# utiasASRL/mm_masking

Hardware: AMD Instinct MI355X
Metric: scan-pairs/s (mask-CNN + 10-iter dICP fwd+bwd) (higher is better)
Workload: dtype bf16; 1 GPU; BASELINE configs[2]: train_icp_weights step fwd+bwd, batch=32 per GPU, 10 dICP iters, point-to-plane Huber, dim=2; 400x3360 polar radar -> GO-CFAR + peaks + polar->Cartesian 640x640 -> U-Net (hand-written NHWC bf16 MFMA kernels, fp32 masters) -> dICP (fp32 points, fp64 normal equations) -> rot+trans+mask_pts loss -> Adam; batch_per_gpu=32, global_batch=32, scan_pts_pad=5120, map_pts=20000, map_pts_pad=20480, icp_iters=10, parallelism=dp1, scene_density=survey (SURVEY.md 8d: 3 500-5 000 valid scan points of 5 120)

## Files before the change

### mm_masking_amd/csrc/mmk_unet.hip

```cpp
#include <math.h>
#include <stdlib.h>

#include <algorithm>
#include <type_traits>

#include "mmk_common.h"
#include "mmk_unet_shared.h"

namespace {

using namespace mmku;

__device__ __forceinline__ unsigned cvt_pk_bf16(float lo, float hi)
{
    unsigned r;
    asm("v_cvt_pk_bf16_f32 %0, %1, %2" : "=v"(r) : "v"(lo), "v"(hi));
    return r;
}
__device__ __forceinline__ unsigned pk_relu_bf16(unsigned x)
{
    unsigned r;
    asm("v_pk_max_i16 %0, %1, 0" : "=v"(r) : "v"(x));
    return r;
}
// ... 670 lines not shown

    float bs8[8];
    if constexpr (C8) {
#pragma unroll
        for (int r = 0; r < 8; ++r) {
            bs8[r] = a.bias ? a.bias[r] : 0.f;
            asm volatile("" : "+v"(bs8[r]));
        }
    }
    const float dk = dp.inv_keep;
    const unsigned thr1pk = ((unsigned)(dp.thr_s - 1 < -32768 ? -32768 : dp.thr_s - 1) & 0xffffu) * 0x00010001u;
#pragma unroll
    for (int m = 0; m < MT; ++m)
#pragma unroll
        for (int r = 0; r < 4; ++r) bs[m][r] *= dk;
    if constexpr (C8) {
#pragma unroll
        for (int r = 0; r < 8; ++r) bs8[r] *= dk;
    }

    MMK_RING_LOAD(0);
    MMK_RING_LOAD(1);
    MMK_RING_SINKS();
    if constexpr (RD > 2) {
        MMK_RING_LOAD(2);
        MMK_RING_SINKS();
    }
    cur_pix0 = s_pix0[0]; cur_ty0 = s_ty0[0]; cur_tx0 = s_tx0[0];
    if constexpr (POOL) cur_pp0 = s_pp0[0];
    MMK_RING_STORE(0, 0);
    MMK_RING_LOAD(0);
    MMK_RING_SINKS();

    int k0 = 0;
    {
#define STAGE_CHECKED 1
#define STAGE_SLOT 0
#include "mmk_conv_ring_stage.inc"
#undef STAGE_SLOT
#define STAGE_SLOT 1
#include "mmk_conv_ring_stage.inc"
#undef STAGE_SLOT
        if constexpr (RD > 2) {
#define STAGE_SLOT 2
#include "mmk_conv_ring_stage.inc"
#undef STAGE_SLOT
        }
#undef STAGE_CHECKED
    }
    for (k0 = RD; k0 + RD <= nt_blk; k0 += RD) {
#define STAGE_CHECKED 0
#define STAGE_SLOT 0
#include "mmk_conv_ring_stage.inc"
#undef STAGE_SLOT
#define STAGE_SLOT 1
#include "mmk_conv_ring_stage.inc"
#undef STAGE_SLOT
        if constexpr (RD > 2) {
#define STAGE_SLOT 2
#include "mmk_conv_ring_stage.inc"
#undef STAGE_SLOT
        }
#undef STAGE_CHECKED
    }
    {
#define STAGE_CHECKED 1
#define STAGE_SLOT 0
#include "mmk_conv_ring_stage.inc"
#undef STAGE_SLOT
        if constexpr (RD > 2) {
#define STAGE_SLOT 1
#include "mmk_conv_ring_stage.inc"
#undef STAGE_SLOT
        }
#undef STAGE_CHECKED
    }
ring_done:;
#ifdef MMK_DEEP_STAMPS
    if (tid == 0) { stamp_lds[16 + 6] = __builtin_amdgcn_s_memtime(); stamp_lds[16 + 7] = __builtin_amdgcn_s_memrealtime(); }
    __syncthreads();
    if (g_deep_stamp_buf != nullptr && blockIdx.y == 0 && blockIdx.x < 4096 && tid == 0) {
        unsigned long long *life = g_deep_stamp_buf + (size_t)64 * (4 * MMK_STAMP_STAGES * 8) + (size_t)blockIdx.x * 2;
        life[0] = stamp_lds[8 + 7];
        life[1] = stamp_lds[16 + 7];
    }
    if (g_deep_stamp_buf != nullptr && blockIdx.y == 0 && blockIdx.x < 64)
        for (int i = tid; i < 4 * MMK_STAMP_STAGES * 8; i += CONV_THREADS)
            g_deep_stamp_buf[(size_t)blockIdx.x * (4 * MMK_STAMP_STAGES * 8) + i] = stamp_lds[i];
#endif
#undef MMK_RING_LOAD
#undef MMK_RING_STORE
}

template <int CK, int CM, int RD, bool EPI, int POOL = 0, bool C8 = false, bool POOLG = false>
int launch_conv_ring(const ConvArgs &a, hipStream_t st)
{
#ifdef MMK_DEEP_STAMPS
    const size_t smem = (((size_t)2 * HT * WT * lds_pitch(CK) + (size_t)ksteps(CK) * (CM / 16) * 512) * sizeof(bf16) + 15) / 16 * 16 +
                        (size_t)4 * MMK_STAMP_STAGES * 8 * sizeof(unsigned long long);
#else
    const size_t smem = ((size_t)2 * HT * WT * lds_pitch(CK) + (size_t)ksteps(CK) * (CM / 16) * 512) * sizeof(bf16);
#endif
    constexpr auto kernel = conv3x3_ring_kernel<CK, CM, RD, EPI, POOL, C8, POOLG>;
    int per_cu = 0;
    MMK_CHECK_HIP(blocks_per_cu<kernel>(CONV_THREADS, smem, 8, &per_cu));
    const int groups = (a.COUT + CM - 1) / CM;
    const XcdGrid g = xcd_grid(a.B, a.H, a.W, TH, TW, groups, per_cu);
    hipLaunchKernelGGL(kernel, dim3(8 * g.nb, groups), dim3(CONV_THREADS), smem, st, a, g.total, g.per_xcd);
    MMK_LAUNCH_CHECK();
    return MMK_OK;
}

inline bool use_c8_epilogue()
{
    static int v = -1;
    if (v < 0) {
        const char *e = getenv("MMK_CONV_C8");
        v = (e && e[0] == '0') ? 0 : 1;
    }
    return v == 1;
}

template <int CK, int CM>
int launch_conv_ring_epi(const ConvArgs &a, hipStream_t st)
{
    constexpr int RD = CK <= 16 ? 3 : 2;
    constexpr int RDE = 2;
    const bool epi = a.o1.relu_src || a.o1.accumulate || (a.o2.C > 0 && (a.o2.relu_src || a.o2.accumulate));
    if (a.x1_pool_arg != nullptr) {
        if constexpr (CK == 32 && CM == 32) {
            if (epi && a.pool_y == nullptr) return launch_conv_ring<CK, CM, RDE, true, 0, false, true>(a, st);
        }
        mmk::set_error("mmk_conv3x3: x1_pool_arg is not supported for this layer (CIN=%d COUT=%d)", a.CIN, a.COUT);
        return MMK_ERR_ARG;
    }
    if (a.pool_y != nullptr) {
        if constexpr (CK == CM && (CK == 16 || CK == 32)) {
            if (!epi && a.o2.C == 0)
                return a.pool_arg != nullptr ? launch_conv_ring<CK, CM, RD, false, 2>(a, st) : launch_conv_ring<CK, CM, RD, false, 1>(a, st);
        }
        mmk::set_error("mmk_conv3x3: pool_y is not supported for this layer (see mmk_conv3x3_pool_fusable)");
        return MMK_ERR_ARG;
    }
    if constexpr (CM == 16) {
        if (a.COUT == 8 && a.o2.C == 0 && use_c8_epilogue())
            return epi ? launch_conv_ring<CK, CM, RDE, true, false, true>(a, st) : launch_conv_ring<CK, CM, RD, false, false, true>(a, st);
    }
    return epi ? launch_conv_ring<CK, CM, RDE, true>(a, st) : launch_conv_ring<CK, CM, RD, false>(a, st);
}


constexpr int DEEP_THREADS = 512;

template <int BM, int NT>
struct DeepCfg {
    static constexpr int WM = BM >= 128 ? 2 : 1;
    static constexpr int WN = 8 / WM;
    static constexpr int MT = BM / 16 / WM;
    static constexpr int MTB = BM / 16;
    static constexpr int TH = WN, TWD = NT * 16;
    static constexpr int HT = TH + 2, WT = TWD + 2;
    static constexpr int CK = 32, PK = 48, NS = 9, GPP = 4;
    static constexpr int NIN = HT * WT * GPP;
    static constexpr int NW = NS * MTB * 64;
    static constexpr int RIN = (NIN + DEEP_THREADS - 1) / DEEP_THREADS;
    static constexpr int RW = (NW + DEEP_THREADS - 1) / DEEP_THREADS;
    static constexpr size_t IN_BYTES = (size_t)HT * WT * PK * sizeof(bf16), W_BYTES = (size_t)NW * 8 * sizeof(bf16);
    static constexpr size_t smem_core(int wchunks) { return IN_BYTES + (size_t)wchunks * W_BYTES + BM * sizeof(float); }
#ifdef MMK_DEEP_STAMPS
    static constexpr size_t smem(int wchunks) { return (smem_core(wchunks) + 15) / 16 * 16 + (size_t)8 * MMK_STAMP_STAGES * 8 * sizeof(unsigned long long); }
#else
    static constexpr size_t smem(int wchunks) { return smem_core(wchunks); }
#endif
};

template <int BM, int NT>
XcdGrid deep_grid(int B, int H, int W, int cout)
{
    return xcd_grid(B, H, W, DeepCfg<BM, NT>::TH, DeepCfg<BM, NT>::TWD, (cout + BM - 1) / BM, 1);
}

template <int BM, int NT, bool LK = false, bool SUBW = false, int ROLE = 0, bool WRES = false, bool POOLG = false>
__global__ __launch_bounds__(DEEP_THREADS) void conv3x3_deep_kernel(const ConvArgs a, int total_tiles, int tiles_per_xcd)
{
    using C = DeepCfg<BM, NT>;
    constexpr int MT = C::MT, MTB = C::MTB, PK = C::PK, WT = C::WT, HT = C::HT, GPP = C::GPP;
    constexpr int NIN = C::NIN, NW = C::NW, RIN = C::RIN, RW = C::RW, NS = C::NS;
    constexpr bool R_FWD = ROLE == 1, R_BWD = ROLE == 2;
    static_assert(!(WRES && SUBW), "resident weights: the kernel's own packing only");
    extern __shared__ __attribute__((aligned(16))) unsigned char smem[];
    bf16 *in_tile = reinterpret_cast<bf16 *>(smem);
    bf16 *w_lds = in_tile + HT * WT * PK;

    const int tid = threadIdx.x, lane = tid & 63, wv = tid >> 6;
    const int wm = wv / C::WN, wn = wv % C::WN;
    const int tiles_x = (a.W + C::TWD - 1) / C::TWD, tiles_y = (a.H + C::TH - 1) / C::TH;
    const int tpi = tiles_x * tiles_y;
    const int group = blockIdx.y;
    const int nchunk = a.CIN / 32;
    const int wchunks = WRES ? nchunk : 1;

    const int xcd = blockIdx.x & 7, nb = gridDim.x >> 3;
    const int t_begin = xcd * tiles_per_xcd;
    const int t_end = (t_begin + tiles_per_xcd < total_tiles) ? t_begin + tiles_per_xcd : total_tiles;
    int tile = t_begin + (blockIdx.x >> 3);
    if (tile >= t_end) return;

    constexpr int RWL = WRES ? 0 : RW;
    constexpr int PHT = C::TH / 2 + 2, PWT = C::TWD / 2 + 2, NPIN = PHT * PWT * GPP;
    constexpr int NRIN = POOLG ? (NPIN + DEEP_THREADS - 1) / DEEP_THREADS : RIN;
    u32x4 rin[NRIN], rw[RW];
    unsigned rcd[POOLG ? NRIN : 1];
    const int Hp = a.H >> 1, Wp = a.W >> 1;
    int g_dy[RIN], g_dx[RIN], g_c[RIN], g_pix[RIN];
#pragma unroll
    for (int i = 0; i < RIN; ++i) {
        int g = tid + i * DEEP_THREADS;
        g = g < NIN ? g : NIN - 1;
        const int pix = g / GPP;
        g_dy[i] = pix / WT - 1;
        g_dx[i] = pix % WT - 1;
        g_c[i] = (g % GPP) * 8;
        g_pix[i] = (pix / WT) * a.W + pix % WT;
        if constexpr (POOLG) {
            int gp = tid + i * DEEP_THREADS;
            gp = gp < NPIN ? gp : NPIN - 1;
            const int pp = gp / GPP;
            g_dy[i] = pp / PWT - 1;
            g_dx[i] = pp % PWT - 1;
            g_c[i] = (gp % GPP) * 8;
            g_pix[i] = g_dy[i] * Wp + g_dx[i];
        }
    }
    const bf16 *ld_base = nullptr;
    int ld_xc = 0, ld_ty0 = 0, ld_tx0 = 0;
    const u32x4 *ld_w = nullptr;
    const unsigned *ld_code = nullptr;
    int ld_moff = 0;
    auto set_stage = [&](int t, int chunk) {
        const int b = t / tpi, tr = t - b * tpi;
        const int tyi = tr / tiles_x;
        ld_tx0 = (tr - tyi * tiles_x) * C::TWD;
        ld_ty0 = tyi * C::TH;
        const int c0 = chunk * 32;
        const bool in1 = c0 < a.C1;
        const bf16 *xb = in1 ? a.x1 : a.x2;
        ld_xc = in1 ? a.C1 : a.C2;
        const int cb = in1 ? c0 : c0 - a.C1;
        const long org = POOLG ? ((long)b * Hp + (ld_ty0 >> 1)) * Wp + (ld_tx0 >> 1)
                               : ((long)b * a.H + ld_ty0 - 1) * a.W + ld_tx0 - 1;
        ld_base = xb + org * ld_xc + cb;
        if constexpr (POOLG) ld_code = a.x1_pool_arg + ((org * ld_xc + cb) >> 3);
        if constexpr (SUBW) {
            const int pm = a.wpack_mtb, per = pm / MTB;
            ld_w = reinterpret_cast<const u32x4 *>(a.wpack + ((size_t)((group / per) * nchunk + chunk)) * NS * pm * 512);
            ld_moff = (group % per) * MTB;
        } else {
            ld_w = reinterpret_cast<const u32x4 *>(a.wpack + ((size_t)(group * nchunk + chunk)) * NW * 8);
        }
    };
    auto issue_in = [&](int i) {
        if constexpr (POOLG) {
            const bool ok = (unsigned)((ld_ty0 >> 1) + g_dy[i]) < (unsigned)Hp && (unsigned)((ld_tx0 >> 1) + g_dx[i]) < (unsigned)Wp;
            const int off = g_pix[i] * ld_xc + g_c[i];
            rin[i] = *(ok ? reinterpret_cast<const u32x4 *>(ld_base + off) : &g_zero16);
            rcd[i] = *(ok ? ld_code + (off >> 3) : reinterpret_cast<const unsigned *>(&g_zero16));
            return;
        }
        const bool ok = (unsigned)(ld_ty0 + g_dy[i]) < (unsigned)a.H && (unsigned)(ld_tx0 + g_dx[i]) < (unsigned)a.W;
        const unsigned off = (unsigned)(g_pix[i] * ld_xc + g_c[i]);
        const u32x4 *sp = ok ? reinterpret_cast<const u32x4 *>(ld_base + off) : &g_zero16;
        rin[i] = *sp;
    };
    auto issue_w = [&](int i) {
        int g = tid + i * DEEP_THREADS;
        g = g < NW ? g : NW - 1;
        if constexpr (SUBW) rw[i] = ld_w[((g / (MTB * 64)) * a.wpack_mtb + ld_moff) * 64 + g % (MTB * 64)];
        else rw[i] = ld_w[g];
    };
    auto write_in = [&]() {
        if constexpr (POOLG) {
#pragma unroll
            for (int i = 0; i < NRIN; ++i) {
                const int g = tid + i * DEEP_THREADS;
                const int r0 = 2 * g_dy[i] + 1, c0 = 2 * g_dx[i] + 1;
                poolg_write(in_tile + (r0 * WT + c0) * PK + g_c[i], PK, WT * PK, r0, c0, HT, WT, g < NPIN, rin[i], rcd[i], a.x1_pool_scale);
            }
            return;
        }
#pragma unroll
        for (int i = 0; i < RIN; ++i) {
            const int g = tid + i * DEEP_THREADS;
            if (g < NIN) *reinterpret_cast<u32x4 *>(in_tile + (size_t)(g / GPP) * PK + (g % GPP) * 8) = rin[i];
        }
    };
    auto write_w = [&](int slot) {
#pragma unroll
        for (int i = 0; i < RW; ++i) {
            const int g = tid + i * DEEP_THREADS;
            if (g < NW) reinterpret_cast<u32x4 *>(w_lds + (size_t)slot * NW * 8)[g] = rw[i];
        }
    };

    const DropoutParams dp = dropout_params(a.drop_p);
    float *bias_lds = reinterpret_cast<float *>(w_lds + (size_t)wchunks * NW * 8);
    if (tid < BM) {
        int c = group * BM + tid;
        if constexpr (SUBW) {
            const int pm = a.wpack_mtb, per = pm / MTB, m_off = (group % per) * MTB;
            c = (group / per) * (pm * 16) + (m_off / 4) * 64 + 16 * (tid / (4 * MT)) + 4 * (m_off % 4) + tid % (4 * MT);
        }
        const float bz = (a.bias && c < a.COUT) ? a.bias[c] : 0.f;
        bias_lds[tid] = R_FWD ? bz * dp.inv_keep : bz;
    }
    f32x4 acc[MT][NT];
    auto reset_acc = [&]() {
#pragma unroll
        for (int m = 0; m < MT; ++m)
#pragma unroll
            for (int n = 0; n < NT; ++n) acc[m][n] = f32x4{0.f, 0.f, 0.f, 0.f};
    };
    reset_acc();

    constexpr bool lk = LK;
    const bf16 *b_base = in_tile + ((size_t)(wn * WT + (lane & 15))) * PK + 8 * (lane >> 4);
    const bf16 *a_base0 = w_lds + ((size_t)(wm * MT) * 64 + lane) * 8;

    int chunk = 0;
#ifdef MMK_DEEP_STAMPS
    unsigned long long *stamp_lds = reinterpret_cast<unsigned long long *>(smem + (C::smem_core(wchunks) + 15) / 16 * 16);
    int stamp_stage = 0;
    for (int i = tid; i < 8 * MMK_STAMP_STAGES * 8; i += DEEP_THREADS) stamp_lds[i] = 0ull;
#endif
    if constexpr (WRES) {
        for (int ck = 0; ck < nchunk; ++ck) {
            set_stage(tile, ck);
#pragma unroll
            for (int i = 0; i < RW; ++i) issue_w(i);
            write_w(ck);
        }
    }
    set_stage(tile, 0);
#pragma unroll
    for (int i = 0; i < NRIN; ++i) issue_in(i);
    if constexpr (!WRES) {
#pragma unroll
        for (int i = 0; i < RW; ++i) issue_w(i);
        write_w(0);
    }
    write_in();
    __syncthreads();

    constexpr int NCH = 4 * MT;
    constexpr int LW = NCH >= 8 ? 8 : 4;
    typedef __attribute__((ext_vector_type(LW))) __bf16 bfl;
    constexpr int NP = NCH / LW;

    while (true) {
        MMK_STAMP(0);
        int ntile = tile, nck = chunk + 1;
        if (nck == nchunk) {
            nck = 0;
            ntile = tile + nb;
        }
        const bool has_next = ntile < t_end;
        set_stage(has_next ? ntile : tile, nck);
        const bf16 *a_base = a_base0 + (WRES ? (size_t)chunk * NW * 8 : (size_t)0);
        MMK_STAMP(1);
#pragma unroll
        for (int s = 0; s < NS; ++s) {
            const int ty = s / 3, tx = s % 3;
            bf16x8 bf[NT];
#pragma unroll
            for (int n = 0; n < NT; ++n)
                bf[n] = *reinterpret_cast<const bf16x8 *>(b_base + ((size_t)(ty * WT + n * 16 + tx)) * PK);
#pragma unroll
            for (int m = 0; m < MT; ++m) {
                const bf16x8 af = *reinterpret_cast<const bf16x8 *>(a_base + ((size_t)(s * MTB + m) * 64) * 8);
#pragma unroll
                for (int n = 0; n < NT; ++n) acc[m][n] = __builtin_amdgcn_mfma_f32_16x16x32_bf16(af, bf[n], acc[m][n], 0, 0, 0);
            }
#pragma unroll
            for (int j = s; j < NRIN + RWL; j += NS) {
                if (j < NRIN) issue_in(j);
                else issue_w(j - NRIN);
            }
            __builtin_amdgcn_sched_barrier(0x38F);
        }
        MMK_STAMP(2);
        auto deliver_and_write = [&]() {
#pragma unroll
            for (int i = 0; i < NRIN; ++i) asm volatile("" : "+v"(rin[i]));
            if constexpr (POOLG) {
#pragma unroll
                for (int i = 0; i < NRIN; ++i) asm volatile("" : "+v"(rcd[i]));
            }
#pragma unroll
            for (int i = 0; i < RWL; ++i) asm volatile("" : "+v"(rw[i]));
            MMK_STAMP(4);
            if (has_next) {
                __syncthreads();
                MMK_STAMP(5);
                write_in();
                if constexpr (!WRES) write_w(0);
            }
            MMK_STAMP(6);
        };
        if (chunk != nchunk - 1) {
            MMK_STAMP(3);
            deliver_and_write();
        } else {
            const int b = tile / tpi, tr = tile - b * tpi;
            const int tyi = tr / tiles_x;
            const int tx0 = (tr - tyi * tiles_x) * C::TWD, yy = tyi * C::TH + wn;
            int lv = lane;
            asm volatile("" : "+v"(lv));
            const int g4 = lv >> 4;
            int c0, e_bias_at;
            if constexpr (SUBW) {
                const int pm = a.wpack_mtb, per = pm / MTB, m_off = (group % per) * MTB;
                c0 = (group / per) * (pm * 16) + (m_off / 4) * 64 + 16 * g4 + 4 * (m_off % 4);
                e_bias_at = NCH * g4;
            } else {
                c0 = group * BM + wm * (16 * MT) + NCH * g4;
                e_bias_at = wm * (16 * MT) + NCH * g4;
            }
            const bool e_on = c0 < a.COUT;
            const bool firstp = c0 < a.o1.C;
            bf16 *const o_y = firstp ? a.o1.y : a.o2.y;
            const bf16 *const o_src = firstp ? a.o1.relu_src : a.o2.relu_src;
            const int o_C = firstp ? a.o1.C : a.o2.C;
            const bool e_acc = (firstp ? a.o1.accumulate : a.o2.accumulate) != 0;
            const float e_scale = firstp ? a.o1.scale : a.o2.scale;
            const int cl = firstp ? c0 : c0 - a.o1.C;
            const int e_x0 = tx0 + (lv & 15);
            const long p0 = ((long)b * a.H + yy) * a.W + e_x0;
            const unsigned e_e0 = (unsigned)p0 * (unsigned)a.COUT + (unsigned)c0 + a.hash_base;
            bf16 *const e_y0 = o_y + p0 * o_C + cl;
            const int e_step = 16 * o_C;
            const bool e_row_ok = yy < a.H;
            const bool e_src = o_src != nullptr;
            const bf16 *const e_pf0 = e_src ? o_src + p0 * o_C + cl : (e_acc ? (const bf16 *)e_y0 : nullptr);
            bfl opnd[R_BWD ? NT : 1][NP];
            auto fetch_operands = [&]() {
#pragma unroll
                for (int n = 0; n < NT; ++n) {
                    const bool okp = e_on && e_pf0 != nullptr && e_row_ok && e_x0 + n * 16 < a.W;
                    const bf16 *pp = okp ? e_pf0 + n * e_step : reinterpret_cast<const bf16 *>(g_zero32);
#pragma unroll
                    for (int k = 0; k < NP; ++k) opnd[R_BWD ? n : 0][k] = *reinterpret_cast<const bfl *>(pp + k * LW);
                }
            };
            if constexpr (R_BWD) fetch_operands();
            if (e_on) {
                if constexpr (R_FWD) {
                    float bk[NCH];
#pragma unroll
                    for (int k = 0; k < NCH; k += 4) {
                        const f32x4 t = *reinterpret_cast<const f32x4 *>(bias_lds + e_bias_at + k);
                        bk[k] = t[0]; bk[k + 1] = t[1]; bk[k + 2] = t[2]; bk[k + 3] = t[3];
                    }
                    const float kf = dp.inv_keep;
                    const int t1s = (int)dp.thr - 32768 - 1;
                    const unsigned t1 = (unsigned)(t1s < -32768 ? -32768 : t1s) & 0xffffu;
                    const unsigned thr1 = t1 | (t1 << 16);
                    const bool drop = dp.thr != 0u;
#pragma unroll
                    for (int n = 0; n < NT; ++n) {
                        const bool okp = e_row_ok && e_x0 + n * 16 < a.W;
                        unsigned hw[MT][2];
#pragma unroll
                        for (int m = 0; m < MT; ++m) hw[m][0] = hw[m][1] = 0x7fff7fffu;
                        if (drop) {
#pragma unroll
                            for (int m = 0; m < MT; ++m)
                                dropout_words(a.seed, e_e0 + (unsigned)n * (16u * (unsigned)a.COUT) + 4u * m, hw[m][0], hw[m][1]);
                        }
                        unsigned pk[NCH / 2];
#pragma unroll
                        for (int m = 0; m < MT; ++m)
#pragma unroll
                            for (int hlf = 0; hlf < 2; ++hlf) {
                                const float t0 = __builtin_fmaf(acc[m][n][2 * hlf], kf, bk[4 * m + 2 * hlf]);
                                const float t1f = __builtin_fmaf(acc[m][n][2 * hlf + 1], kf, bk[4 * m + 2 * hlf + 1]);
                                pk[2 * m + hlf] = pk_relu_bf16(cvt_pk_bf16(t0, t1f)) & pk_keep_mask(hw[m][hlf], thr1);
                            }
                        bf16 *const dst = okp ? e_y0 + n * e_step : reinterpret_cast<bf16 *>(g_sink32);
                        if constexpr (NCH >= 8) {
#pragma unroll
                            for (int k = 0; k < NCH / 2; k += 4)
                                *reinterpret_cast<u32x4 *>(dst + 2 * k) = (u32x4){pk[k], pk[k + 1], pk[k + 2], pk[k + 3]};
                        } else {
                            *reinterpret_cast<unsigned long long *>(dst) = ((unsigned long long)pk[1] << 32) | pk[0];
                        }
                        __builtin_amdgcn_sched_barrier(0);
                    }
                } else {
                    float bv[NCH];
                    if constexpr (!R_BWD) {
#pragma unroll
                        for (int k = 0; k < NCH; k += 4) {
                            const f32x4 t = *reinterpret_cast<const f32x4 *>(bias_lds + e_bias_at + k);
                            bv[k] = t[0]; bv[k + 1] = t[1]; bv[k + 2] = t[2]; bv[k + 3] = t[3];
                        }
                    }
                    const bool o_accf = !e_src && e_acc;
#pragma unroll
                    for (int n = 0; n < NT; ++n) {
                        const bool okp = e_row_ok && e_x0 + n * 16 < a.W;
                        float v[NCH];
#pragma unroll
                        for (int m = 0; m < MT; ++m)
#pragma unroll
                            for (int r = 0; r < 4; ++r) {
                                float t = acc[m][n][r];
                                if constexpr (!R_BWD) {
                                    t += bv[4 * m + r];
                                    if (a.relu) t = lk ? act_leaky(t, a.slope) : fmaxf(t, 0.f);
                                }
                                v[4 * m + r] = t;
                            }
                        if constexpr (!R_BWD) {
                            if (dp.thr != 0u) {
#pragma unroll
                                for (int m = 0; m < MT; ++m) {
                                    float sc[4];
                                    dropout_scale4(a.seed, e_e0 + (unsigned)n * (16u * (unsigned)a.COUT) + 4u * m, dp, sc);
#pragma unroll
                                    for (int r = 0; r < 4; ++r) v[4 * m + r] = lk ? drop_leaky(v[4 * m + r], sc[r]) : v[4 * m + r] * sc[r];
                                }
                            }
                        }
                        bf16 *const dst0 = e_y0 + n * e_step;
                        if constexpr (R_BWD) {
                            if (e_pf0 != nullptr && okp) {
                                if (!o_accf) {
#pragma unroll
                                    for (int k = 0; k < NCH; k += LW) {
                                        const bfl sv = opnd[n][k / LW];
#pragma unroll
                                        for (int r = 0; r < LW; ++r) v[k + r] = ((float)sv[r] > 0.f) ? v[k + r] * e_scale : 0.f;
                                    }
                                } else {
#pragma unroll
                                    for (int k = 0; k < NCH; k += LW) {
                                        const bfl ov = opnd[n][k / LW];
#pragma unroll
                                        for (int r = 0; r < LW; ++r) v[k + r] += (float)ov[r];
                                    }
                                }
                            }
                        } else {
                            if (e_src && okp) {
                                const bf16 *sp = e_pf0 + n * e_step;
#pragma unroll
                                for (int k = 0; k < NCH; k += LW) {
                                    const bfl sv = *reinterpret_cast<const bfl *>(sp + k);
#pragma unroll
                                    for (int r = 0; r < LW; ++r)
                                        v[k + r] = lk ? v[k + r] * bwd_factor_leaky((float)sv[r], e_scale, a.slope)
                                                      : (((float)sv[r] > 0.f) ? v[k + r] * e_scale : 0.f);
                                }
                            }
                            if (e_acc && okp) {
#pragma unroll
                                for (int k = 0; k < NCH; k += LW) {
                                    const bfl ov = *reinterpret_cast<const bfl *>(dst0 + k);
#pragma unroll
                                    for (int r = 0; r < LW; ++r) v[k + r] += (float)ov[r];
                                }
                            }
                        }
                        if (R_BWD || okp) {
                            bf16 *const dst = (R_BWD && !okp) ? reinterpret_cast<bf16 *>(g_sink32) : dst0;
                            if constexpr (NCH >= 8) {
#pragma unroll
                                for (int k = 0; k < NCH; k += 8) {
                                    bf16x8 o8;
#pragma unroll
                                    for (int r = 0; r < 8; ++r) o8[r] = (bf16)v[k + r];
                                    *reinterpret_cast<bf16x8 *>(dst + k) = o8;
                                }
                            } else {
                                bf16x4 o4;
#pragma unroll
                                for (int r = 0; r < 4; ++r) o4[r] = (bf16)v[r];
                                *reinterpret_cast<bf16x4 *>(dst) = o4;
                            }
                        }
                    }
                }
            }
            reset_acc();
            MMK_STAMP(3);
            deliver_and_write();
        }
        if (!has_next) break;
        __syncthreads();
        MMK_STAMP(7);
#ifdef MMK_DEEP_STAMPS
        ++stamp_stage;
#endif
        tile = ntile;
        chunk = nck;
    }
#ifdef MMK_DEEP_STAMPS
    __syncthreads();
    if (g_deep_stamp_buf != nullptr && blockIdx.y == 0 && blockIdx.x < 64)
        for (int i = tid; i < 8 * MMK_STAMP_STAGES * 8; i += DEEP_THREADS)
            g_deep_stamp_buf[(size_t)blockIdx.x * (8 * MMK_STAMP_STAGES * 8) + i] = stamp_lds[i];
#endif
}

template <int BM, int NT, bool LK = false, bool SUBW = false, int ROLE = 0, bool WRES = false, bool POOLG = false>
int launch_conv_deep(const ConvArgs &a, hipStream_t st)
{
    using C = DeepCfg<BM, NT>;
    constexpr auto kernel = conv3x3_deep_kernel<BM, NT, LK, SUBW, ROLE, WRES, POOLG>;
    MMK_CHECK_HIP(raise_lds_limit<kernel>(true, 160 * 1024));
    const size_t smem = C::smem(WRES ? a.CIN / 32 : 1);
    MMK_REQUIRE(smem <= (size_t)160 * 1024, "mmk_conv3x3: %zu bytes of LDS for CIN=%d COUT=%d", smem, a.CIN, a.COUT);
    const XcdGrid g = deep_grid<BM, NT>(a.B, a.H, a.W, a.COUT);
    hipLaunchKernelGGL(kernel, dim3(8 * g.nb, (a.COUT + BM - 1) / BM), dim3(DEEP_THREADS), smem, st, a, g.total, g.per_xcd);
    MMK_LAUNCH_CHECK();
    return MMK_OK;
}

template <int BM, int NT>
bool deep_weights_fit(int cin) { return DeepCfg<BM, NT>::smem(cin / 32) <= (size_t)160 * 1024; }

template <class F>
int with_deep_cfg(int BM, bool narrow, F &&f)
{
    return with_int<16, 32, 64, 128>(BM, [&](auto M) {
        return narrow ? f(M, std::integral_constant<int, 3>{}) : f(M, std::integral_constant<int, 5>{});
    });
}

int deep_rounds(int B, int H, int W, int cout, int BM, bool narrow, int *tiles_per_image)
{
    return with_deep_cfg(BM, narrow, [&](auto M, auto NT) {
        const XcdGrid g = deep_grid<M(), NT()>(B, H, W, cout);
        if (tiles_per_image) *tiles_per_image = g.tiles;
        return g.rounds();
    });
}

int dispatch_conv_deep_plain(const ConvArgs &a, hipStream_t st);

int dispatch_conv_deep(const ConvArgs &a, hipStream_t st)
{
    const int BM = conv_cm(a.CIN, a.COUT);
    const bool narrow = a.W <= 48;
    const char *split_env = getenv("MMK_CONV_SPLIT");
    const bool split_on = !(split_env && split_env[0] == '0');
    int tpi = 0;
    const bool forward_role = a.relu != 0 && a.o1.relu_src == nullptr && a.o2.relu_src == nullptr && !a.o1.accumulate && !a.o2.accumulate;
    if (split_on && forward_role && a.slope == 0.f && (BM == 64 || BM == 128) && a.COUT % 32 == 0 && a.pool_y == nullptr && a.wpack_mtb == 0 &&
        deep_rounds(a.B, a.H, a.W, a.COUT, BM, narrow, &tpi) == 2) {
        const int groups = (a.COUT + BM - 1) / BM, nb = std::max(1, 32 / groups);
        const int Bm = (8 * nb) / tpi;
        const int Bt = a.B - Bm;
        const bool under_filled = (long)a.B * tpi * groups * 10 < (long)256 * 2 * 7;
        if (Bm >= 1 && Bt >= 1 && under_filled && deep_rounds(Bm, a.H, a.W, a.COUT, BM, narrow, nullptr) == 1 &&
            deep_rounds(Bt, a.H, a.W, a.COUT, 32, narrow, nullptr) == 1 && (a.o1.C % 32 == 0) && (a.o2.C % 32 == 0)) {
            ConvArgs m = a;
            m.B = Bm;
            int rc = dispatch_conv_deep_plain(m, st);
            if (rc != MMK_OK) return rc;
            ConvArgs t = a;
            const size_t px = (size_t)Bm * a.H * a.W;
            t.B = Bt;
            t.x1 = a.x1 + px * a.C1;
            if (a.x2) t.x2 = a.x2 + px * a.C2;
            auto adv = [&](ConvOutPart &o) {
                if (o.y) o.y += px * o.C;
                if (o.relu_src) o.relu_src += px * o.C;
            };
            adv(t.o1);
            adv(t.o2);
            t.hash_base = a.hash_base + (unsigned)(px * a.COUT);
            t.wpack_mtb = BM / 16;
            return narrow ? launch_conv_deep<32, 3, false, true, 1>(t, st) : launch_conv_deep<32, 5, false, true, 1>(t, st);
        }
    }
    return dispatch_conv_deep_plain(a, st);
}

int dispatch_conv_deep_plain(const ConvArgs &a, hipStream_t st)
{
    const bool any_src = a.o1.relu_src != nullptr || (a.o2.C > 0 && a.o2.relu_src != nullptr);
    const bool any_acc = a.o1.accumulate != 0 || (a.o2.C > 0 && a.o2.accumulate != 0);
    const bool both1 = a.o1.relu_src != nullptr && a.o1.accumulate != 0, both2 = a.o2.C > 0 && a.o2.relu_src != nullptr && a.o2.accumulate != 0;
    const int role = (a.relu != 0 && !any_src && !any_acc) ? 1
                   : ((a.relu == 0 && a.bias == nullptr && dropout_params(a.drop_p).thr == 0u && !both1 && !both2) ? 2 : 0);
    const int rc = with_deep_cfg(conv_cm(a.CIN, a.COUT), a.W <= 48, [&](auto M, auto N) -> int {
        constexpr int BM = M(), NT = N();
        constexpr bool WRES = BM <= 64;
        const bool resident = WRES && a.wpack_mtb == 0 && deep_weights_fit<BM, NT>(a.CIN);
        if (a.slope > 0.f) return launch_conv_deep<BM, NT, true>(a, st);
        if (a.x1_pool_arg != nullptr) {
            if constexpr (BM >= 64) {
                if (role == 2 && a.wpack_mtb == 0) {
                    if (resident) return launch_conv_deep<BM, NT, false, false, 2, WRES, true>(a, st);
                    if (BM > 64) return launch_conv_deep<BM, NT, false, false, 2, false, true>(a, st);
                }
            }
            mmk::set_error("mmk_conv3x3: x1_pool_arg is not supported for this layer (CIN=%d COUT=%d)", a.CIN, a.COUT);
            return MMK_ERR_ARG;
        }
        if constexpr (BM >= 32) {
            if (role == 1) return resident ? launch_conv_deep<BM, NT, false, false, 1, WRES>(a, st) : launch_conv_deep<BM, NT, false, false, 1>(a, st);
            if (role == 2) return resident ? launch_conv_deep<BM, NT, false, false, 2, WRES>(a, st) : launch_conv_deep<BM, NT, false, false, 2>(a, st);
        }
        return launch_conv_deep<BM, NT>(a, st);
    });
    if (rc != NO_KERNEL) return rc;
    mmk::set_error("mmk_conv3x3: unsupported channel counts CIN=%d COUT=%d", a.CIN, a.COUT);
    return MMK_ERR_ARG;
}

bool pool_fusable(int cin, int cout, int B, int H, int W)
{
    const bool fits32 = (size_t)B * H * W * (size_t)std::max(cin, cout) < ((size_t)1 << 31);
    return cin == cout && (cin == 16 || cin == 32) && fits32 && H >= 2 && W >= 2;
}

template <class F>
int with_thin_shape(int CK, int CM, F &&f)
{
    return with_int<8, 16, 32>(CK, [&](auto K) {
        return with_int<16, 32, 64>(CM, [&](auto M) {
            if constexpr (K() == 32 && M() == 64) return NO_KERNEL;
            else return f(K, M);
        });
    });
}

int dispatch_conv(const ConvArgs &a, hipStream_t st)
{
    if (a.pool_y != nullptr && (a.slope > 0.f || !pool_fusable(a.CIN, a.COUT, a.B, a.H, a.W))) {
        mmk::set_error("mmk_conv3x3: pool_y is not supported for this layer (see mmk_conv3x3_pool_fusable)");
        return MMK_ERR_ARG;
    }
    if (a.x1_pool_arg != nullptr && (a.slope > 0.f || a.C2 != 0 || a.H < 2 || a.W < 2)) {
        mmk::set_error("mmk_conv3x3: x1_pool_arg needs the ReLU network, a single input and H, W >= 2");
        return MMK_ERR_ARG;
    }
    if (conv_is_deep(a.CIN, a.COUT)) {
        if (a.o2.C > 0 && conv_cm(a.CIN, a.COUT) >= 64 && a.o1.C % 16 != 0) {
            mmk::set_error("mmk_conv3x3: output split %d+%d: layers of >= 64 output channels split at multiples of 16", a.o1.C, a.o2.C);
            return MMK_ERR_ARG;
        }
        return dispatch_conv_deep(a, st);
    }
    const int CK = conv_ck(a.CIN), CM = conv_cm(a.CIN, a.COUT);
    if (a.x1_pool_arg != nullptr && !(a.CIN == 32 && CM == 32 && (size_t)a.B * a.H * a.W * 32 < ((size_t)1 << 31))) {
        mmk::set_error("mmk_conv3x3: x1_pool_arg is not supported for this layer (CIN=%d COUT=%d)", a.CIN, a.COUT);
        return MMK_ERR_ARG;
    }
    const bool fits32 = (size_t)a.B * a.H * a.W * (size_t)std::max(a.CIN, a.COUT) < ((size_t)1 << 31);
    const bool ring = a.CIN == CK && CM <= 32 && fits32;
    const int rc = with_thin_shape(CK, CM, [&](auto K, auto M) -> int {
        if (a.slope > 0.f) return launch_conv<K(), M(), true>(a, st);
        if constexpr (M() <= 32) {
            if (ring) return launch_conv_ring_epi<K(), M()>(a, st);
        }
        return launch_conv<K(), M()>(a, st);
    });
    if (rc != NO_KERNEL) return rc;
    mmk::set_error("mmk_conv3x3: unsupported channel counts CIN=%d COUT=%d", a.CIN, a.COUT);
    return MMK_ERR_ARG;
}


typedef __attribute__((ext_vector_type(2))) int i32x2;
typedef __attribute__((ext_vector_type(4))) int i32x4;

__device__ __forceinline__ unsigned lds_addr(const void *p)
{
    return (unsigned)(size_t)(__attribute__((address_space(3))) const void *)p;
}

__device__ __forceinline__ i32x2 tr_read(unsigned addr)
{
    i32x2 v;
    asm volatile("ds_read_b64_tr_b16 %0, %1" : "=v"(v) : "v"(addr) : "memory");
    return v;
}

template <int OFF>
__device__ __forceinline__ i32x2 tr_read_o(unsigned addr)
{
    static_assert(OFF >= 0 && OFF < 65536, "ds offset field is 16 bits");
    i32x2 v;
    asm volatile("ds_read_b64_tr_b16 %0, %1 offset:%2" : "=v"(v) : "v"(addr), "n"(OFF) : "memory");
    return v;
}

__device__ __forceinline__ bf16x8 frag_from(i32x2 lo, i32x2 hi)
{
    i32x4 t = {lo.x, lo.y, hi.x, hi.y};
    return __builtin_bit_cast(bf16x8, t);
}

struct WgradArgs {
    const bf16 *x1, *x2;
    int C1, C2;
    const bf16 *g;
    int B, H, W, CIN, COUT;
    float *partials;
    int acc_partials;
    const unsigned *g_arg = nullptr;
    float g_scale = 1.f;
};

template <int CK, int CM, bool G8, bool POOLG = false>
__global__ __launch_bounds__(CONV_THREADS) void conv3x3_wgrad_kernel(const WgradArgs a)
{
    constexpr int MT = CM / 16;
    constexpr int NTT = (CK >= 16) ? 9 * (CK / 16) : 5;
    constexpr int NTW = (NTT + 3) / 4;
    extern __shared__ __attribute__((aligned(16))) unsigned char smem[];
    constexpr int PK = wg_pitch(CK);
    constexpr int GCOLS = G8 ? 8 : CM;
    constexpr int PG = wg_pitch(GCOLS);
    bf16 *x_tile = reinterpret_cast<bf16 *>(smem);
    bf16 *g_tile = x_tile + (HT * WT + 8) * PK;

    const int tid = threadIdx.x, lane = tid & 63;
    const int wv = __builtin_amdgcn_readfirstlane(tid >> 6);
    const int chunk = blockIdx.y, group = blockIdx.z;
    const int tiles_x = (a.W + TW - 1) / TW, tiles_y = (a.H + TH - 1) / TH;
    const int tpi = tiles_x * tiles_y;
    const int total_tiles = tpi * a.B;
    const int i16 = lane & 15, g4 = lane >> 4, q = i16 >> 2, pp = i16 & 3;

    f32x4 acc[MT][NTW];
    f32x4 accb[MT];
#pragma unroll
    for (int m = 0; m < MT; ++m) {
        accb[m] = (f32x4){0.f, 0.f, 0.f, 0.f};
#pragma unroll
        for (int n = 0; n < NTW; ++n) acc[m][n] = (f32x4){0.f, 0.f, 0.f, 0.f};
    }
    bf16x8 ones;
#pragma unroll
    for (int j = 0; j < 8; ++j) ones[j] = (bf16)1.0f;
// ... 2834 lines not shown
```

Baseline: 3542 pairs/s.

## Add co-resident deep conv variant with two blocks per CU for narrow layers

Adds a variant of the deep 3x3 conv kernel (BM=64, NT=3, streamed sub-weights) with a trimmed input halo width, so each block stays within 80 KB of LDS and two blocks fit on one CU. It also requests four waves per EU. Index precomputation arrays are dropped in favour of recomputing offsets on the fly, which lowers register pressure. Weight loads are deferred to the deliver phase. The variant is enabled by default for BM=128 layers with width up to 44 in both forward and backward roles, with an env knob to turn it off. The trade-off is more per-load index arithmetic and smaller output tiles per block in exchange for higher occupancy and latency hiding.

```diff
diff --git a/mm_masking_amd/csrc/mmk_unet.hip b/mm_masking_amd/csrc/mmk_unet.hip
--- a/mm_masking_amd/csrc/mmk_unet.hip
+++ b/mm_masking_amd/csrc/mmk_unet.hip
@@ -846,14 +846,14 @@
 
 constexpr int DEEP_THREADS = 512;
 
-template <int BM, int NT>
+template <int BM, int NT, int HW = 0>
 struct DeepCfg {
     static constexpr int WM = BM >= 128 ? 2 : 1;
     static constexpr int WN = 8 / WM;
     static constexpr int MT = BM / 16 / WM;
     static constexpr int MTB = BM / 16;
     static constexpr int TH = WN, TWD = NT * 16;
-    static constexpr int HT = TH + 2, WT = TWD + 2;
+    static constexpr int HT = TH + 2, WT = HW > 0 ? HW : TWD + 2;
     static constexpr int CK = 32, PK = 48, NS = 9, GPP = 4;
     static constexpr int NIN = HT * WT * GPP;
     static constexpr int NW = NS * MTB * 64;
@@ -874,10 +874,13 @@
     return xcd_grid(B, H, W, DeepCfg<BM, NT>::TH, DeepCfg<BM, NT>::TWD, (cout + BM - 1) / BM, 1);
 }
 
-template <int BM, int NT, bool LK = false, bool SUBW = false, int ROLE = 0, bool WRES = false, bool POOLG = false>
-__global__ __launch_bounds__(DEEP_THREADS) void conv3x3_deep_kernel(const ConvArgs a, int total_tiles, int tiles_per_xcd)
-{
-    using C = DeepCfg<BM, NT>;
+template <int BM, int NT, bool LK = false, bool SUBW = false, int ROLE = 0, bool WRES = false, bool POOLG = false, int HW = 0>
+__global__ __launch_bounds__(DEEP_THREADS) __attribute__((amdgpu_waves_per_eu(HW > 0 ? 4 : 2, HW > 0 ? 4 : 8)))
+void conv3x3_deep_kernel(const ConvArgs a, int total_tiles, int tiles_per_xcd)
+{
+    static_assert(HW == 0 || (BM == 64 && NT == 3 && SUBW && !LK && DeepCfg<BM, NT, HW>::smem_core(1) <= (size_t)80 * 1024),
+                  "two blocks per CU: 80 KB of LDS each");
+    using C = DeepCfg<BM, NT, HW>;
     constexpr int MT = C::MT, MTB = C::MTB, PK = C::PK, WT = C::WT, HT = C::HT, GPP = C::GPP;
     constexpr int NIN = C::NIN, NW = C::NW, RIN = C::RIN, RW = C::RW, NS = C::NS;
     constexpr bool R_FWD = ROLE == 1, R_BWD = ROLE == 2;
@@ -900,15 +903,19 @@
     int tile = t_begin + (blockIdx.x >> 3);
     if (tile >= t_end) return;
 
+    constexpr bool CO = HW > 0;
     constexpr int RWL = WRES ? 0 : RW;
+    constexpr int RWE = CO ? 0 : RWL;
     constexpr int PHT = C::TH / 2 + 2, PWT = C::TWD / 2 + 2, NPIN = PHT * PWT * GPP;
     constexpr int NRIN = POOLG ? (NPIN + DEEP_THREADS - 1) / DEEP_THREADS : RIN;
     u32x4 rin[NRIN], rw[RW];
     unsigned rcd[POOLG ? NRIN : 1];
     const int Hp = a.H >> 1, Wp = a.W >> 1;
-    int g_dy[RIN], g_dx[RIN], g_c[RIN], g_pix[RIN];
-#pragma unroll
-    for (int i = 0; i < RIN; ++i) {
+    static_assert(!CO || (!POOLG && !WRES), "co-resident blocks: streamed weights, plain input");
+    constexpr int NG = CO ? 1 : RIN;
+    int g_dy[NG], g_dx[NG], g_c[NG], g_pix[NG];
+#pragma unroll
+    for (int i = 0; i < (CO ? 0 : RIN); ++i) {
         int g = tid + i * DEEP_THREADS;
         g = g < NIN ? g : NIN - 1;
         const int pix = g / GPP;
@@ -953,6 +960,14 @@
             ld_w = reinterpret_cast<const u32x4 *>(a.wpack + ((size_t)(group * nchunk + chunk)) * NW * 8);
         }
     };
+    auto otid = [&]() {
+        int t = tid;
+        if constexpr (CO) {
+            asm volatile("" : "+v"(t));
+            t &= DEEP_THREADS - 1;
+        }
+        return t;
+    };
     auto issue_in = [&](int i) {
         if constexpr (POOLG) {
             const bool ok = (unsigned)((ld_ty0 >> 1) + g_dy[i]) < (unsigned)Hp && (unsigned)((ld_tx0 >> 1) + g_dx[i]) < (unsigned)Wp;
@@ -961,13 +976,23 @@
             rcd[i] = *(ok ? ld_code + (off >> 3) : reinterpret_cast<const unsigned *>(&g_zero16));
             return;
         }
+        if constexpr (CO) {
+            const int t = otid();
+            int pix = (t >> 2) + i * (DEEP_THREADS / GPP);
+            pix = pix < HT * WT ? pix : HT * WT - 1;
+            const int row = pix / WT, col = pix - row * WT;
+            const bool ok = (unsigned)(ld_ty0 + row - 1) < (unsigned)a.H && (unsigned)(col - 1) < (unsigned)a.W;
+            const unsigned off = (unsigned)((row * a.W + col) * ld_xc + (t & 3) * 8);
+            rin[i] = *(ok ? reinterpret_cast<const u32x4 *>(ld_base + off) : &g_zero16);
+            return;
+        }
         const bool ok = (unsigned)(ld_ty0 + g_dy[i]) < (unsigned)a.H && (unsigned)(ld_tx0 + g_dx[i]) < (unsigned)a.W;
         const unsigned off = (unsigned)(g_pix[i] * ld_xc + g_c[i]);
         const u32x4 *sp = ok ? reinterpret_cast<const u32x4 *>(ld_base + off) : &g_zero16;
         rin[i] = *sp;
     };
     auto issue_w = [&](int i) {
-        int g = tid + i * DEEP_THREADS;
+        int g = otid() + i * DEEP_THREADS;
         g = g < NW ? g : NW - 1;
         if constexpr (SUBW) rw[i] = ld_w[((g / (MTB * 64)) * a.wpack_mtb + ld_moff) * 64 + g % (MTB * 64)];
         else rw[i] = ld_w[g];
@@ -982,16 +1007,18 @@
             }
             return;
         }
+        const int wt = otid();
 #pragma unroll
         for (int i = 0; i < RIN; ++i) {
-            const int g = tid + i * DEEP_THREADS;
+            const int g = wt + i * DEEP_THREADS;
             if (g < NIN) *reinterpret_cast<u32x4 *>(in_tile + (size_t)(g / GPP) * PK + (g % GPP) * 8) = rin[i];
         }
     };
     auto write_w = [&](int slot) {
+        const int wt = otid();
 #pragma unroll
         for (int i = 0; i < RW; ++i) {
-            const int g = tid + i * DEEP_THREADS;
+            const int g = wt + i * DEEP_THREADS;
             if (g < NW) reinterpret_cast<u32x4 *>(w_lds + (size_t)slot * NW * 8)[g] = rw[i];
         }
     };
@@ -1075,7 +1102,7 @@
                 for (int n = 0; n < NT; ++n) acc[m][n] = __builtin_amdgcn_mfma_f32_16x16x32_bf16(af, bf[n], acc[m][n], 0, 0, 0);
             }
 #pragma unroll
-            for (int j = s; j < NRIN + RWL; j += NS) {
+            for (int j = s; j < NRIN + RWE; j += NS) {
                 if (j < NRIN) issue_in(j);
                 else issue_w(j - NRIN);
             }
@@ -1083,6 +1110,10 @@
         }
         MMK_STAMP(2);
         auto deliver_and_write = [&]() {
+            if constexpr (CO) {
+#pragma unroll
+                for (int i = 0; i < RWL; ++i) issue_w(i);
+            }
 #pragma unroll
             for (int i = 0; i < NRIN; ++i) asm volatile("" : "+v"(rin[i]));
             if constexpr (POOLG) {
@@ -1090,7 +1121,7 @@
                 for (int i = 0; i < NRIN; ++i) asm volatile("" : "+v"(rcd[i]));
             }
 #pragma unroll
-            for (int i = 0; i < RWL; ++i) asm volatile("" : "+v"(rw[i]));
+            for (int i = 0; i < RWE; ++i) asm volatile("" : "+v"(rw[i]));
             MMK_STAMP(4);
             if (has_next) {
                 __syncthreads();
@@ -1285,9 +1316,10 @@
                     }
                 }
             }
-            reset_acc();
+            if constexpr (!CO) reset_acc();
             MMK_STAMP(3);
             deliver_and_write();
+            if constexpr (CO) reset_acc();
         }
         if (!has_next) break;
         __syncthreads();
@@ -1320,6 +1352,21 @@
     return MMK_OK;
 }
 
+template <int HW, int ROLE>
+int launch_conv_deep_cores(const ConvArgs &a, hipStream_t st, bool flat)
+{
+    constexpr int CORES_BM = 64, CORES_NT = 3;
+    using C = DeepCfg<CORES_BM, CORES_NT, HW>;
+    constexpr auto kernel = conv3x3_deep_kernel<CORES_BM, CORES_NT, false, true, ROLE, false, false, HW>;
+    MMK_CHECK_HIP(raise_lds_limit<kernel>(true, C::smem(1)));
+    const int groups = (a.COUT + CORES_BM - 1) / CORES_BM;
+    XcdGrid g = xcd_grid(a.B, a.H, a.W, C::TH, C::TWD, groups, 2);
+    if (flat && g.rounds() > 1) g.nb = g.per_xcd;
+    hipLaunchKernelGGL(kernel, dim3(8 * g.nb, groups), dim3(DEEP_THREADS), C::smem(1), st, a, g.total, g.per_xcd);
+    MMK_LAUNCH_CHECK();
+    return MMK_OK;
+}
+
 template <int BM, int NT>
 bool deep_weights_fit(int cin) { return DeepCfg<BM, NT>::smem(cin / 32) <= (size_t)160 * 1024; }
 
@@ -1342,10 +1389,35 @@
 
 int dispatch_conv_deep_plain(const ConvArgs &a, hipStream_t st);
 
+int deep_role(const ConvArgs &a)
+{
+    const bool any_src = a.o1.relu_src != nullptr || (a.o2.C > 0 && a.o2.relu_src != nullptr);
+    const bool any_acc = a.o1.accumulate != 0 || (a.o2.C > 0 && a.o2.accumulate != 0);
+    const bool both1 = a.o1.relu_src != nullptr && a.o1.accumulate != 0, both2 = a.o2.C > 0 && a.o2.relu_src != nullptr && a.o2.accumulate != 0;
+    return (a.relu != 0 && !any_src && !any_acc) ? 1
+         : ((a.relu == 0 && a.bias == nullptr && dropout_params(a.drop_p).thr == 0u && !both1 && !both2) ? 2 : 0);
+}
+
+int dispatch_conv_deep_cores(const ConvArgs &a, hipStream_t st)
+{
+    const char *env = getenv("MMK_DEEP_CORES");
+    const int mode = (env == nullptr || env[0] < '0' || env[0] > '3') ? 1 : env[0] - '0';
+    const int role = deep_role(a);
+    const bool serves = conv_cm(a.CIN, a.COUT) == 128 && a.COUT % 64 == 0 && a.W <= 44 && a.slope == 0.f && a.pool_y == nullptr &&
+                        a.wpack_mtb == 0 && a.x1_pool_arg == nullptr && (role == 1 || role == 2);
+    if (mode == 0 || !serves || (mode == 3 && role != 1)) return NO_KERNEL;
+    const bool flat = mode != 2;
+    ConvArgs t = a;
+    t.wpack_mtb = 8;
+    if (a.W <= 40) return role == 1 ? launch_conv_deep_cores<42, 1>(t, st, flat) : launch_conv_deep_cores<42, 2>(t, st, flat);
+    return role == 1 ? launch_conv_deep_cores<46, 1>(t, st, flat) : launch_conv_deep_cores<46, 2>(t, st, flat);
+}
+
 int dispatch_conv_deep(const ConvArgs &a, hipStream_t st)
 {
     const int BM = conv_cm(a.CIN, a.COUT);
     const bool narrow = a.W <= 48;
+    if (const int rc = dispatch_conv_deep_cores(a, st); rc != NO_KERNEL) return rc;
     const char *split_env = getenv("MMK_CONV_SPLIT");
     const bool split_on = !(split_env && split_env[0] == '0');
     int tpi = 0;
@@ -1383,11 +1455,7 @@
 
 int dispatch_conv_deep_plain(const ConvArgs &a, hipStream_t st)
 {
-    const bool any_src = a.o1.relu_src != nullptr || (a.o2.C > 0 && a.o2.relu_src != nullptr);
-    const bool any_acc = a.o1.accumulate != 0 || (a.o2.C > 0 && a.o2.accumulate != 0);
-    const bool both1 = a.o1.relu_src != nullptr && a.o1.accumulate != 0, both2 = a.o2.C > 0 && a.o2.relu_src != nullptr && a.o2.accumulate != 0;
-    const int role = (a.relu != 0 && !any_src && !any_acc) ? 1
-                   : ((a.relu == 0 && a.bias == nullptr && dropout_params(a.drop_p).thr == 0u && !both1 && !both2) ? 2 : 0);
+    const int role = deep_role(a);
     const int rc = with_deep_cfg(conv_cm(a.CIN, a.COUT), a.W <= 48, [&](auto M, auto N) -> int {
         constexpr int BM = M(), NT = N();
         constexpr bool WRES = BM <= 64;
```

Result: no change. 3555 pairs/s, median of 6 (+0.4%).
